# ablab/spades

Hardware: NVIDIA H100
Metric: Mk-mers/s (extract+count+index) k=55, 150 bp reads (higher is better)
Workload: dtype u64

## Files before the change

spades_b200/csrc/count.cu:

```cuda
#include <time.h>

#include <algorithm>
#include <type_traits>

#include "sgpu_internal.h"

namespace sg {

struct ReadsSrc {
    const uint64_t *words;
    const uint64_t *offs;
    const uint32_t *lens;
    int64_t n;
    uint64_t nwords;
    int K;
    int both;
    __device__ __forceinline__ uint32_t nrec(int64_t item) const {
        int L = (int)lens[item];
        uint32_t w = L >= K ? (uint32_t)(L - K + 1) : 0u;
        return both ? 2u * w : w;
    }
    template <int NW, typename Ptr>
    __device__ __forceinline__ Kmer<NW> get_at(Ptr s, uint32_t j) const {
        uint32_t pos = both ? (j >> 1) : j;
// ... 285 lines not shown
        __syncthreads();
    }
    for (uint32_t i = threadIdx.x; i < p.PA; i += blockDim.x) mybase[i] = cur_base[i] + cnt[i];
}

static const int kRollC = 24;
static_assert(kRollC <= 33 && kRollC % 8 == 0, "roll_init fetches a chunk's bases from two words; an id row is a whole number of 16-byte words");
static const int kRollThreads = 512;

static const int kRollTile = 32;
static const int kRollWarps = kRollThreads / 32;
static const int kRollStageWords = 320;
__device__ __forceinline__ void prefetch_l2(const void *p) { asm volatile("prefetch.global.L2 [%0];" ::"l"(p)); }
struct RollWarp {
    uint64_t words[kRollStageWords];
    uint32_t pref[kRollTile + 1];
    uint32_t len[kRollTile];
    uint32_t off[kRollTile];
    uint32_t pad_;
};
static_assert(sizeof(RollWarp) % 8 == 0, "per-warp slices stay 8-byte aligned");
static size_t roll_smem_bytes(uint32_t nslots) { return (((size_t)nslots * 4 + 15) & ~(size_t)15) + (size_t)kRollWarps * sizeof(RollWarp); }
__device__ __forceinline__ RollWarp *roll_warp_slice(unsigned char *raw, uint32_t nslots) {
    return reinterpret_cast<RollWarp *>(raw + (((size_t)nslots * 4 + 15) & ~(size_t)15)) + (threadIdx.x >> 5);
}

__device__ __forceinline__ uint32_t roll_warp_setup(const ReadsSrc &src, int64_t item0, int nitems, RollWarp &rw, uint32_t *uniform, bool *staged) {
    const int lane = threadIdx.x & 31;
    uint32_t c = 0, L = 0;
    uint64_t a = 0, b = 0;
    if (lane < nitems) {
        L = src.lens[item0 + lane];
        a = src.offs[item0 + lane];
        b = a + (((uint64_t)L + 31) >> 5);
        const uint32_t w = (int)L >= src.K ? (uint32_t)((int)L - src.K + 1) : 0u;
        c = (w + kRollC - 1) / kRollC;
    }
    uint32_t inc = c;
#pragma unroll
    for (int o = 1; o < 32; o <<= 1) {
        const uint32_t t = __shfl_up_sync(0xffffffffu, inc, o);
        if (lane >= o) inc += t;
    }
    rw.len[lane] = L;
    rw.pref[lane] = inc - c;
    const uint32_t total = __shfl_sync(0xffffffffu, inc, 31);
    if (lane == 31) rw.pref[kRollTile] = total;
    const uint32_t c0 = __shfl_sync(0xffffffffu, c, 0);
    const bool same = __all_sync(0xffffffffu, lane >= nitems || c == c0);
    *uniform = (same && c0) ? c0 : 0u;
    const uint64_t w0 = __shfl_sync(0xffffffffu, a, 0);
    const bool ok = lane >= nitems || (a >= w0 && b >= a && b - w0 <= (uint64_t)kRollStageWords);
    const bool st = __all_sync(0xffffffffu, ok);
    if (st) {
        rw.off[lane] = (uint32_t)(a - w0);
        uint32_t end = lane < nitems ? (uint32_t)(b - w0) : 0u;
#pragma unroll
        for (int o = 16; o; o >>= 1) end = max(end, __shfl_xor_sync(0xffffffffu, end, o));
        uint64_t tmp[kRollStageWords / 32];
#pragma unroll
        for (int j = 0; j < kRollStageWords / 32; ++j) tmp[j] = (uint32_t)(lane + 32 * j) < end ? __ldg(src.words + w0 + lane + 32 * j) : 0ull;
#pragma unroll
        for (int j = 0; j < kRollStageWords / 32; ++j) if ((uint32_t)(lane + 32 * j) < end) rw.words[lane + 32 * j] = tmp[j];
    }
    *staged = st;
    __syncwarp();
    return total;
}

__global__ void roll_tile_ids_k(ReadsSrc src, int64_t ntiles, uint32_t *__restrict__ out) {
    const int64_t t = (int64_t)blockIdx.x * (blockDim.x >> 5) + (threadIdx.x >> 5);
    if (t >= ntiles) return;
    const int lane = threadIdx.x & 31;
    const int64_t item = t * kRollTile + lane;
    uint32_t s = 0;
    if (item < src.n) {
        const int L = (int)src.lens[item];
        const uint32_t w = L >= src.K ? (uint32_t)(L - src.K + 1) : 0u;
        s = (w + kRollC - 1) / kRollC;
    }
    for (int o = 16; o; o >>= 1) s += __shfl_down_sync(0xffffffffu, s, o);
    if (lane == 0) out[t] = s * kRollC;
}

struct RollUnit { int it, j0, cnt; };
__device__ __forceinline__ RollUnit roll_unit(const RollWarp &rw, int nitems, uint32_t u, uint32_t unif, int K) {
    RollUnit q;
    q.it = find_item_u(rw.pref, nitems, u, unif);
    q.j0 = (int)(u - rw.pref[q.it]) * kRollC;
    const int nwin = (int)rw.len[q.it] - K + 1;
    q.cnt = nwin - q.j0 < kRollC ? nwin - q.j0 : kRollC;
    return q;
}

template <int NW>
__global__ void __launch_bounds__(kRollThreads, 2) levelA_count_roll_k(ReadsSrc src, LevelA p, uint32_t *__restrict__ blk_counts,
                                                                      const uint64_t *__restrict__ tile_off, uint16_t *__restrict__ ids) {
    extern __shared__ __align__(16) unsigned char sm_raw[];
    uint32_t *hist = reinterpret_cast<uint32_t *>(sm_raw);
    RollWarp &rw = *roll_warp_slice(sm_raw, p.PA);
    for (uint32_t i = threadIdx.x; i < p.PA; i += blockDim.x) hist[i] = 0;
    __syncthreads();
    const int K = p.K;
    const int lane = threadIdx.x & 31, warp = threadIdx.x >> 5;
    const int64_t ntiles = (src.n + kRollTile - 1) / kRollTile;
    const int64_t per = (ntiles + gridDim.x - 1) / gridDim.x;
    const int64_t t0 = (int64_t)blockIdx.x * per, t1 = min(ntiles, t0 + per);
    for (int64_t t = t0 + warp; t < t1; t += kRollWarps) {
        const int64_t item0 = t * kRollTile;
        const int nitems = (int)min((int64_t)kRollTile, src.n - item0);
        uint32_t unif = 0;
        bool staged = false;
        const bool has_next = t + kRollWarps < t1;
        const int64_t nx = (t + kRollWarps) * kRollTile;
        uint64_t next_w0 = 0;
        if (has_next) {
            next_w0 = src.offs[nx];
            if (lane == 0) prefetch_l2(src.lens + nx);
            else if (lane == 1 && nx + 16 < src.n) prefetch_l2(src.offs + nx + 16);
        }
        const uint32_t nunits = roll_warp_setup(src, item0, nitems, rw, &unif, &staged);
        uint64_t *row = ids ? reinterpret_cast<uint64_t *>(ids + tile_off[t]) : nullptr;
        for (uint32_t u = lane; u < nunits; u += 32) {
            const RollUnit q = roll_unit(rw, nitems, u, unif, K);
            const uint64_t *seq = staged ? static_cast<const uint64_t *>(rw.words + rw.off[q.it]) : src.words + src.offs[item0 + q.it];
            RollState<NW> st;
            roll_init<NW>(st, seq, q.j0, K, q.cnt);
#pragma unroll 1
            for (int g = 0; g < kRollC / 4; ++g) {
                uint64_t acc = 0;
#pragma unroll
                for (int e = 0; e < 4; ++e) {
                    const int s = 4 * g + e;
                    uint32_t id = 0xffffu;
                    if (s < q.cnt) {
                        if (s > 0) roll_next<NW>(st, K);
                        const Kmer<NW> k = kmer_is_minimal<NW>(st.f, st.r) ? st.f : st.r;
                        uint32_t part;
                        if (part_of<NW>(p, k, &part)) { atomicAdd(&hist[part], 1u); id = part; }
                    }
                    acc |= (uint64_t)id << (16 * e);
                }
                if (row) row[(size_t)u * (kRollC / 4) + g] = acc;
            }
        }
        if (has_next && lane < 10 && next_w0 + 16 * lane < src.nwords) prefetch_l2(src.words + next_w0 + 16 * lane);
        __syncwarp();
    }
    __syncthreads();
    uint32_t *out = blk_counts + (size_t)blockIdx.x * p.PA;
    for (uint32_t i = threadIdx.x; i < p.PA; i += blockDim.x) out[i] += hist[i];
}

template <int NW, bool HAS_IDS>
__global__ void __launch_bounds__(kRollThreads, 2) levelA_scatter_roll_k(ReadsSrc src, LevelA p, uint64_t *__restrict__ base, uint64_t *__restrict__ out,
                                                                        const uint64_t *__restrict__ tile_off, const uint16_t *__restrict__ ids,
                                                                        uint32_t id_lo, uint32_t row_stride, uint32_t q_lo, uint64_t ids_len) {
    extern __shared__ __align__(16) unsigned char sm_raw[];
    uint32_t *cur = reinterpret_cast<uint32_t *>(sm_raw);
    RollWarp &rw = *roll_warp_slice(sm_raw, p.PA);
    uint64_t *mybase = base + (size_t)blockIdx.x * row_stride + q_lo;
    const uint64_t region0 = mybase[0];
    for (uint32_t i = threadIdx.x; i < p.PA; i += blockDim.x) cur[i] = (uint32_t)(mybase[i] - region0);
    __syncthreads();
    uint64_t *const out0 = out + region0 * NW;
    const int K = p.K;
    const uint32_t PA = p.PA;
    const int lane = threadIdx.x & 31, warp = threadIdx.x >> 5;
    const int64_t ntiles = (src.n + kRollTile - 1) / kRollTile;
    const int64_t per = (ntiles + gridDim.x - 1) / gridDim.x;
    const int64_t t0 = (int64_t)blockIdx.x * per, t1 = min(ntiles, t0 + per);
    for (int64_t t = t0 + warp; t < t1; t += kRollWarps) {
        const int64_t item0 = t * kRollTile;
        const int nitems = (int)min((int64_t)kRollTile, src.n - item0);
        uint32_t unif = 0;
        bool staged = false;
        const bool has_next = t + kRollWarps < t1;
        const int64_t nx = (t + kRollWarps) * kRollTile;
        uint64_t next_w0 = 0;
        if (has_next) {
            next_w0 = src.offs[nx];
            if (lane == 0) prefetch_l2(src.lens + nx);
            else if (lane == 1 && nx + 16 < src.n) prefetch_l2(src.offs + nx + 16);
        }
        uint64_t next_row = 0;
        if (HAS_IDS && has_next) next_row = tile_off[t + kRollWarps];
        const uint32_t nunits = roll_warp_setup(src, item0, nitems, rw, &unif, &staged);
        const ulonglong2 *row = HAS_IDS ? reinterpret_cast<const ulonglong2 *>(ids + tile_off[t]) : nullptr;
        for (uint32_t u = lane; u < nunits; u += 32) {
            uint64_t idw[kRollC / 4];
            if (HAS_IDS) {
#pragma unroll
                for (int v = 0; v < kRollC / 8; ++v) {
                    const ulonglong2 x = __ldg(row + (size_t)u * (kRollC / 8) + v);
                    idw[2 * v] = x.x; idw[2 * v + 1] = x.y;
                }
            }
            const RollUnit q = roll_unit(rw, nitems, u, unif, K);
            const uint64_t *seq = staged ? static_cast<const uint64_t *>(rw.words + rw.off[q.it]) : src.words + src.offs[item0 + q.it];
            RollState<NW> st;
            roll_init<NW>(st, seq, q.j0, K, q.cnt);
#pragma unroll
            for (int s = 0; s < kRollC; ++s) {
                if (s >= q.cnt) break;
                if (s > 0) roll_next<NW>(st, K);
                uint32_t part;
                bool mine;
                if (HAS_IDS) {
                    part = (uint32_t)((idw[s >> 2] >> (16 * (s & 3))) & 0xffffu) - id_lo;
                    mine = part < PA;
                    if (mine) {
                        const uint32_t slot = atomicAdd(&cur[part], 1u);
                        const bool fwd = kmer_is_minimal<NW>(st.f, st.r);
                        Kmer<NW> k;
#pragma unroll
                        for (int j = 0; j < NW; ++j) k.w[j] = fwd ? st.f.w[j] : st.r.w[j];
                        store_rec_stream<NW>(out0 + (size_t)slot * NW, k);
                    }
                } else {
                    const Kmer<NW> k = kmer_is_minimal<NW>(st.f, st.r) ? st.f : st.r;
                    mine = part_of<NW>(p, k, &part);
                    if (mine) {
                        const uint32_t slot = atomicAdd(&cur[part], 1u);
                        store_rec_stream<NW>(out0 + (size_t)slot * NW, k);
                    }
                }
            }
        }
        if (has_next && lane < 10 && next_w0 + 16 * lane < src.nwords) prefetch_l2(src.words + next_w0 + 16 * lane);
        if (HAS_IDS && has_next) {
            if (next_row + 64 * lane < ids_len) prefetch_l2(ids + next_row + 64 * lane);
            if (lane < 16 && next_row + 64 * (32 + lane) < ids_len) prefetch_l2(ids + next_row + 64 * (32 + lane));
        }
        __syncwarp();
    }
    __syncthreads();
    for (uint32_t i = threadIdx.x; i < PA; i += blockDim.x) mybase[i] = region0 + cur[i];
}


struct Seg {
    uint64_t start;
    uint64_t len;
    uint32_t bits;
    uint32_t bb;
};

__global__ void seg_init_k(const uint64_t *__restrict__ part_start, const uint64_t *__restrict__ part_total, uint32_t PA, int rA,
                           uint32_t b_lo, Seg *__restrict__ segs) {
    uint32_t part = blockIdx.x * blockDim.x + threadIdx.x;
    if (part >= PA) return;
    Seg s;
    s.start = part_start[part]; s.len = part_total[part]; s.bits = (uint32_t)rA; s.bb = ((b_lo + (part >> rA)) << 1) | 0u;
    segs[part] = s;
}

struct Pieces {
    const uint64_t *pbase;
    const uint32_t *cnt;
    uint32_t cnt_stride, PA;
    int G;
};
static const int kMaxPieces = 1024;

__global__ void stage_rows_k(const uint32_t *__restrict__ cnt, uint32_t cnt_stride, uint32_t PA, uint64_t *__restrict__ rel, uint64_t *__restrict__ row_total) {
    __shared__ uint64_t wsum[8];
    __shared__ uint64_t carry_s;
    const uint32_t *row = cnt + (size_t)blockIdx.x * cnt_stride;
    uint64_t *out = rel + (size_t)blockIdx.x * PA;
    const int lane = threadIdx.x & 31, warp = threadIdx.x >> 5;
    if (threadIdx.x == 0) carry_s = 0;
    __syncthreads();
    for (uint32_t b = 0; b < PA; b += blockDim.x) {
        const uint32_t i = b + threadIdx.x;
        const uint64_t v = i < PA ? row[i] : 0;
        uint64_t inc = v;
#pragma unroll
        for (int o = 1; o < 32; o <<= 1) {
            uint64_t t = __shfl_up_sync(0xffffffffu, inc, o);
            if (lane >= o) inc += t;
        }
        if (lane == 31) wsum[warp] = inc;
        __syncthreads();
        uint64_t wb = 0, all = 0;
        for (int w = 0; w < 8; ++w) { if (w < warp) wb += wsum[w]; all += wsum[w]; }
        const uint64_t carry = carry_s;
        if (i < PA) out[i] = carry + wb + inc - v;
        __syncthreads();
        if (threadIdx.x == 0) carry_s = carry + all;
        __syncthreads();
    }
    if (threadIdx.x == 0) row_total[blockIdx.x] = carry_s;
}
__global__ void stage_add_k(uint64_t *__restrict__ rel, const uint64_t *__restrict__ row_start, uint32_t PA, int G) {
    const uint64_t i = (uint64_t)blockIdx.x * blockDim.x + threadIdx.x;
    if (i >= (uint64_t)G * PA) return;
    rel[i] += row_start[i / PA];
}

struct RefinePlan { uint32_t cap, target, rmax; int total_bits; };
__device__ __forceinline__ int plan_r(const RefinePlan &rp, uint64_t len, uint32_t bits) {
    if (len <= rp.cap) return 0;
    int rem = rp.total_bits - (int)bits;
    if (rem <= 0) return 0;
    uint64_t want = (len + rp.target - 1) / rp.target;
    int r = 1;
    while (r < (int)rp.rmax && (1ull << r) < want) ++r;
    return r < rem ? r : rem;
}
__global__ void refine_plan_k(const Seg *__restrict__ segs, uint64_t n, RefinePlan rp, uint32_t *__restrict__ nchild, uint32_t *__restrict__ isw, int force_all) {
    uint64_t i = (uint64_t)blockIdx.x * blockDim.x + threadIdx.x;
    if (i >= n) return;
    int r = plan_r(rp, segs[i].len, segs[i].bits);
    nchild[i] = r ? (1u << r) : 1u;
    isw[i] = (r || force_all) ? 1u : 0u;
}
__global__ void refine_copy_k(const Seg *__restrict__ segs, uint64_t n, const uint32_t *__restrict__ isw, const uint64_t *__restrict__ child_base,
                              const uint64_t *__restrict__ work_pos, Seg *__restrict__ nsegs, uint64_t *__restrict__ worklist) {
    uint64_t i = (uint64_t)blockIdx.x * blockDim.x + threadIdx.x;
    if (i >= n) return;
    if (isw[i]) worklist[work_pos[i]] = i;
    else nsegs[child_base[i]] = segs[i];
}

static const int kRThreads = 1024;
static const int kRWarps = kRThreads / 32;
static const int kRMaxBins = 2048;
template <int NW> struct RBatch {
    static const int RPT = NW == 1 ? 12 : NW == 2 ? 8 : NW == 3 ? 4 : 3;
    static const int N = RPT * kRThreads;
    static constexpr size_t smem() { return (size_t)N * (NW * sizeof(uint64_t) + sizeof(uint32_t)); }
};

template <int NW, bool PIECED>
__global__ void __launch_bounds__(kRThreads) refine_k(const Seg *__restrict__ segs, const uint64_t *__restrict__ worklist, uint64_t nwork,
                                                     const uint64_t *__restrict__ child_base, RefinePlan rp, int K,
                                                     uint64_t *__restrict__ buf0, uint64_t *__restrict__ buf1, Seg *__restrict__ nsegs,
                                                     unsigned long long *__restrict__ work_counter, Pieces pc) {
    constexpr int RPT = RBatch<NW>::RPT, N = RBatch<NW>::N;
    __shared__ uint32_t hist[kRMaxBins];
    __shared__ uint32_t run_off[kRMaxBins];
    __shared__ uint32_t run_slot[kRMaxBins];
    __shared__ uint32_t warp_tot[kRWarps];
    __shared__ unsigned long long s_w;
    __shared__ uint64_t pc_start[PIECED ? kMaxPieces : 1];
    __shared__ uint32_t pc_len[PIECED ? kMaxPieces : 1];
    extern __shared__ uint64_t sm_refine_dyn[];
    uint64_t *stage = sm_refine_dyn;
    uint32_t *stage_slot = reinterpret_cast<uint32_t *>(stage + (size_t)N * NW);
    const int lane = threadIdx.x & 31, warp = threadIdx.x >> 5;
    for (;;) {
        if (threadIdx.x == 0) s_w = atomicAdd(work_counter, 1ull);
        __syncthreads();
        const uint64_t wi = s_w;
        __syncthreads();
        if (wi >= nwork) return;
        const uint64_t si = worklist[wi];
        const Seg s = segs[si];
        const int r = plan_r(rp, s.len, s.bits);
        const uint32_t nb = 1u << r;
        const uint64_t *src = ((s.bb & 1) ? buf1 : buf0) + s.start * NW;
        uint64_t *dst = ((s.bb & 1) ? buf0 : buf1) + s.start * NW;
        if (PIECED) {
            for (int g = threadIdx.x; g < pc.G; g += blockDim.x) {
                pc_start[g] = pc.pbase[(size_t)g * pc.PA + si];
                pc_len[g] = pc.cnt[(size_t)g * pc.cnt_stride + si];
            }
        }
        for (uint32_t i = threadIdx.x; i < nb; i += blockDim.x) hist[i] = 0;
        __syncthreads();
        if (PIECED) {
            for (int g = warp; g < pc.G; g += kRWarps) {
                const uint64_t *ps = buf0 + pc_start[g] * NW;
                const uint32_t n = pc_len[g];
                uint32_t i = lane;
                for (; i + 96 < n; i += 128) {
                    const Kmer<NW> k0 = load_rec<NW>(ps + (uint64_t)i * NW), k1 = load_rec<NW>(ps + (uint64_t)(i + 32) * NW);
                    const Kmer<NW> k2 = load_rec<NW>(ps + (uint64_t)(i + 64) * NW), k3 = load_rec<NW>(ps + (uint64_t)(i + 96) * NW);
                    atomicAdd(&hist[key_bits<NW>(k0, K, (int)s.bits, r)], 1u);
                    atomicAdd(&hist[key_bits<NW>(k1, K, (int)s.bits, r)], 1u);
                    atomicAdd(&hist[key_bits<NW>(k2, K, (int)s.bits, r)], 1u);
                    atomicAdd(&hist[key_bits<NW>(k3, K, (int)s.bits, r)], 1u);
                }
                for (; i < n; i += 32) {
                    const Kmer<NW> k = load_rec<NW>(ps + (uint64_t)i * NW);
                    atomicAdd(&hist[key_bits<NW>(k, K, (int)s.bits, r)], 1u);
                }
            }
        } else {
            for (uint64_t i = threadIdx.x; i < s.len; i += blockDim.x) {
                Kmer<NW> k = load_rec<NW>(src + i * NW);
                atomicAdd(&hist[key_bits<NW>(k, K, (int)s.bits, r)], 1u);
// ... 478 lines not shown
        if (const char *e = getenv("SGPU_RMAX")) x.rmax = (uint32_t)std::min(11, std::max(1, atoi(e)));
        if (const char *e = getenv("SGPU_A_SUB")) x.a_sub = std::min(64, std::max(0, atoi(e)));
        x.trace = getenv("SGPU_TRACE") != nullptr;
        return x;
    }();
    return t;
}

struct Trace {
    bool on; cudaStream_t st; double t0;
    static double now() { struct timespec ts; clock_gettime(CLOCK_MONOTONIC, &ts); return ts.tv_sec * 1e3 + ts.tv_nsec * 1e-6; }
    Trace(cudaStream_t s) : on(tuning().trace), st(s), t0(now()) {}
    void mark(const char *what) {
        if (!on) return;
        cudaStreamSynchronize(st);
        double t = now();
        fprintf(stderr, "[sgpu-trace] %-28s %9.3f ms\n", what, t - t0);
        t0 = t;
    }
};

static int ilog2_floor(uint64_t v) { int r = 0; while (v >>= 1) ++r; return r; }

static const int kLevelAMaxParts = 8192;

template <int NW> static uint32_t sort_target() { return (uint32_t)SortCfg<NW>::CAP * 6 / 8; }

template <int NW>
static void sort_pass(Ctx *ctx, int K, DArr<uint64_t> &X, DArr<uint64_t> &Y, const uint64_t *part_start_p, const uint64_t *part_total_p, uint32_t PA,
                      int rA_, uint32_t b_lo, int b_hi, int64_t first, bool want_counts, bool double_selfrc, unsigned long long *d_bsz_p, Chunk &ch_out,
                      Timer &tm, Trace &tr, const Pieces *pieces = nullptr) {
    constexpr int CAP = SortCfg<NW>::CAP;
    const int total_bits = 2 * K;
    cudaStream_t st = ctx->stream;
    uint64_t nsegs = PA;
    DArr<Seg> segs(ctx, nsegs);
    seg_init_k<<<div_up(PA, 256), 256, 0, st>>>(part_start_p, part_total_p, PA, rA_, b_lo, segs.p);
    ctx->launches++;
    RefinePlan rp; rp.cap = CAP; rp.target = sort_target<NW>(); rp.total_bits = total_bits;
    rp.rmax = tuning().rmax;
    DArr<unsigned long long> wcounter(ctx, 4);
    tm.start();
    uint64_t rounds = 0;
    for (int round = 0; round < 300; ++round) {
        DArr<uint32_t> nchild(ctx, nsegs + 1), isw(ctx, nsegs + 1);
        DArr<uint64_t> cbase(ctx, nsegs + 1), wpos(ctx, nsegs + 1);
        SG_CUDA(cudaMemsetAsync(nchild.p + nsegs, 0, 4, st));
        SG_CUDA(cudaMemsetAsync(isw.p + nsegs, 0, 4, st));
        const bool pieced = pieces && round == 0;
        refine_plan_k<<<div_up(nsegs, 256), 256, 0, st>>>(segs.p, nsegs, rp, nchild.p, isw.p, pieced ? 1 : 0);
        ctx->launches++;
        exclusive_scan_u32_to_u64(ctx, nchild.p, cbase.p, nsegs + 1);
        exclusive_scan_u32_to_u64(ctx, isw.p, wpos.p, nsegs + 1);
        uint64_t tot[2];
        SG_CUDA(cudaMemcpyAsync(&tot[0], cbase.p + nsegs, 8, cudaMemcpyDeviceToHost, st));
        SG_CUDA(cudaMemcpyAsync(&tot[1], wpos.p + nsegs, 8, cudaMemcpyDeviceToHost, st));
        SG_CUDA(cudaStreamSynchronize(st));
        if (tot[1] == 0) break;
        DArr<Seg> nsegs_arr(ctx, tot[0]);
        DArr<uint64_t> worklist(ctx, tot[1]);
        refine_copy_k<<<div_up(nsegs, 256), 256, 0, st>>>(segs.p, nsegs, isw.p, cbase.p, wpos.p, nsegs_arr.p, worklist.p);
        ctx->launches++;
        SG_CUDA(cudaMemsetAsync(wcounter.p, 0, 8, st));
        const int grid = (int)std::min<uint64_t>(tot[1], (uint64_t)ctx->num_sms);
        const size_t sm = RBatch<NW>::smem();
        if (pieced) {
            SG_CUDA(cudaFuncSetAttribute(refine_k<NW, true>, cudaFuncAttributeMaxDynamicSharedMemorySize, (int)sm));
            refine_k<NW, true><<<grid, kRThreads, sm, st>>>(segs.p, worklist.p, tot[1], cbase.p, rp, K, X.p, Y.p, nsegs_arr.p, wcounter.p, *pieces);
        } else {
            SG_CUDA(cudaFuncSetAttribute(refine_k<NW, false>, cudaFuncAttributeMaxDynamicSharedMemorySize, (int)sm));
            refine_k<NW, false><<<grid, kRThreads, sm, st>>>(segs.p, worklist.p, tot[1], cbase.p, rp, K, X.p, Y.p, nsegs_arr.p, wcounter.p, Pieces());
        }
        ctx->launches++;
        SG_CUDA(cudaGetLastError());
        tr.mark("refine round");
        (round == 0 ? ctx->times.refine_splits_round0 : ctx->times.refine_splits_later) += tot[0] - nsegs;
        ++rounds;
        segs = std::move(nsegs_arr);
        nsegs = tot[0];
    }
    ctx->times.refine_rounds_max = std::max(ctx->times.refine_rounds_max, rounds);
    ctx->times.refine += tm.stop();
    DArr<uint32_t> ndist(ctx, nsegs + 1);
    DArr<unsigned long long> stats(ctx, 4);
    SG_CUDA(cudaMemsetAsync(ndist.p, 0, ndist.bytes(), st));
    SG_CUDA(cudaMemsetAsync(stats.p, 0, 32, st));
    SG_CUDA(cudaMemsetAsync(wcounter.p, 0, 8, st));
    tm.start();
    {
        auto launch = [&](auto kernel, size_t smem) {
            SG_CUDA(cudaFuncSetAttribute(kernel, cudaFuncAttributeMaxDynamicSharedMemorySize, (int)smem));
            int occ = 1;
            SG_CUDA(cudaOccupancyMaxActiveBlocksPerMultiprocessor(&occ, kernel, kSThreads, smem));
            if (occ < 1) occ = 1;
            int grid = (int)std::min<uint64_t>(nsegs, (uint64_t)ctx->num_sms * occ);
            if (grid < 1) grid = 1;
            kernel<<<grid, kSThreads, smem, st>>>(segs.p, nsegs, K, X.p, Y.p, ndist.p, wcounter.p, stats.p);
        };
        constexpr int bins = 1 << kSortBinBits;
        launch(local_sort3_k<NW, kSortBinBits, CAP>, (size_t)(CAP + kResCap) * NW * sizeof(uint64_t) + (size_t)3 * bins * sizeof(uint32_t) +
                                                         ((size_t)2 * bins + 2 + kResCap) * sizeof(uint16_t) + 16);
        ctx->launches++;
        SG_CUDA(cudaGetLastError());
    }
    DArr<uint64_t> dbase(ctx, nsegs + 1);
    exclusive_scan_u32_to_u64(ctx, ndist.p, dbase.p, nsegs + 1);
    uint64_t D = 0;
    unsigned long long h_stats[4];
    SG_CUDA(cudaMemcpyAsync(&D, dbase.p + nsegs, 8, cudaMemcpyDeviceToHost, st));
    SG_CUDA(cudaMemcpyAsync(h_stats, stats.p, 32, cudaMemcpyDeviceToHost, st));
    SG_CUDA(cudaStreamSynchronize(st));
    ctx->times.local_sort += tm.stop();
    tr.mark("local sort");
    SG_CHECK(h_stats[0] == 0, 6, "internal: oversize segment with unfixed key bits reached the local sort");
    ctx->times.sort_lsd_fallbacks += h_stats[1];
    ctx->times.sort_oversize_equal += h_stats[2];
    Chunk ch;
    ch.n = (int64_t)D; ch.b_lo = (int)b_lo; ch.b_hi = b_hi; ch.first = first;
    ch.keys.alloc(ctx, (size_t)D * NW + 2, true);
    if (want_counts) ch.counts.alloc(ctx, (size_t)D + 1, true);
    tm.start();
    if (nsegs) {
        compact_k<NW><<<div_up((int64_t)nsegs * 32, 256), 256, 0, st>>>(segs.p, nsegs, ndist.p, dbase.p, X.p, Y.p, K, want_counts ? 1 : 0,
                                                                     double_selfrc ? 1 : 0, ch.keys.p, ch.counts.p, d_bsz_p);
        ctx->launches++;
        SG_CUDA(cudaGetLastError());
    }
    ctx->times.compact += tm.stop();
    tr.mark("compact");
    ch_out = std::move(ch);
}

template <int NW, class Src>
struct LevelAJob {
    Ctx *ctx = nullptr;
    std::vector<Src> srcs;
    int K = 0, B = 0, rA = 0, G = 0;
    int s_lo = 0, s_hi = 0;
    uint32_t PA_all = 0;
    bool roll = false, use_ids = false;
    DArr<uint32_t> blk_counts;
    DArr<uint64_t> part_total_all;
    std::vector<DArr<uint64_t>> tile_off;
    std::vector<DArr<uint16_t>> ids;
    std::vector<uint64_t> h_part;
    uint64_t bucket_records(int b) const {
        uint64_t s = 0;
        for (uint32_t q = 0; q < (1u << rA); ++q) s += h_part[((size_t)(b - s_lo) << rA) + q];
        return s;
    }
};

static int levelA_ctas_per_sm() { return 2; }
static int levelA_key_bits(uint64_t est_records, int B, int total_bits, uint32_t target, uint32_t pa_max) {
    const int want = ilog2_floor(est_records / target + 1) + 1;
    const int bbits = ilog2_floor((uint64_t)B) + (((1u << ilog2_floor((uint64_t)B)) < (uint32_t)B) ? 1 : 0);
    int rA = want - bbits;
    if (rA < 0) rA = 0;
    while (rA > 0 && ((uint64_t)B << rA) > pa_max) --rA;
    if (rA > total_bits) rA = total_bits;
    if (rA > 13) rA = 13;
    return rA;
}

template <int NW, class Src>
static void levelA_count(LevelAJob<NW, Src> &job, uint64_t est_records, Timer &tm, Trace &tr) {
    Ctx *ctx = job.ctx;
    cudaStream_t st = ctx->stream;
    const uint32_t PA_all = job.PA_all;
    const int G = job.G;
    SG_CHECK(PA_all >= 1 && PA_all <= (uint32_t)kLevelAMaxParts, 6, "internal: level-A partition table too large");
    LevelA pa_all;
    pa_all.K = job.K; pa_all.B = (uint32_t)job.B; pa_all.b_lo = (uint32_t)job.s_lo; pa_all.b_hi = (uint32_t)job.s_hi; pa_all.rA = job.rA; pa_all.PA = PA_all;
    job.blk_counts.alloc(ctx, (size_t)G * PA_all);
    job.part_total_all.alloc(ctx, (size_t)PA_all + 1);
    job.h_part.assign(PA_all, 0);
    SG_CUDA(cudaMemsetAsync(job.blk_counts.p, 0, job.blk_counts.bytes(), st));
    job.tile_off.clear(); job.ids.clear();
    job.tile_off.resize(job.srcs.size()); job.ids.resize(job.srcs.size());
    job.use_ids = PA_all < 0xffffu && (double)est_records * 2.0 < (double)ctx->free_bytes() * 0.20;
    if (job.use_ids) {
        for (size_t si = 0; si < job.srcs.size(); ++si) {
            const Src &src = job.srcs[si];
            if (src.n == 0) continue;
            const int64_t ntiles = (src.n + (job.roll ? kRollTile : kATile) - 1) / (job.roll ? kRollTile : kATile);
            DArr<uint32_t> ttot(ctx, (size_t)ntiles + 1);
            job.tile_off[si].alloc(ctx, (size_t)ntiles + 1);
            SG_CUDA(cudaMemsetAsync(ttot.p + ntiles, 0, 4, st));
            if (job.roll) {
                if constexpr (std::is_same<Src, ReadsSrc>::value) roll_tile_ids_k<<<div_up(ntiles, 8), 256, 0, st>>>(src, ntiles, ttot.p);
            } else {
                tile_totals_k<Src><<<div_up(ntiles, 8), 256, 0, st>>>(src, ntiles, ttot.p, 8u);
            }
            ctx->launches++;
            exclusive_scan_u32_to_u64(ctx, ttot.p, job.tile_off[si].p, (size_t)ntiles + 1);
            uint64_t nrec_src = 0;
            SG_CUDA(cudaMemcpyAsync(&nrec_src, job.tile_off[si].p + ntiles, 8, cudaMemcpyDeviceToHost, st));
            SG_CUDA(cudaStreamSynchronize(st));
            job.ids[si].alloc(ctx, (size_t)nrec_src + 8);
        }
    }
    tm.start();
    for (size_t si = 0; si < job.srcs.size(); ++si) {
        const Src &src = job.srcs[si];
        if (src.n == 0) continue;
        if (job.roll) {
            if constexpr (std::is_same<Src, ReadsSrc>::value) {
                SG_CUDA(cudaFuncSetAttribute(levelA_count_roll_k<NW>, cudaFuncAttributeMaxDynamicSharedMemorySize, (int)roll_smem_bytes(PA_all)));
                levelA_count_roll_k<NW><<<G, kRollThreads, roll_smem_bytes(PA_all), st>>>(src, pa_all, job.blk_counts.p, job.tile_off[si].p, job.ids[si].p);
            }
        } else {
            SG_CUDA(cudaFuncSetAttribute(levelA_count_k<NW, Src>, cudaFuncAttributeMaxDynamicSharedMemorySize, (int)(PA_all * sizeof(uint32_t))));
            levelA_count_k<NW, Src><<<G, kAThreads, PA_all * sizeof(uint32_t), st>>>(src, pa_all, job.blk_counts.p, job.tile_off[si].p, job.ids[si].p);
        }
        ctx->launches++;
    }
    SG_CUDA(cudaGetLastError());
    levelA_totals_k<<<div_up(PA_all, 256), 256, 0, st>>>(job.blk_counts.p, PA_all, G, job.part_total_all.p);
    ctx->launches++;
    SG_CUDA(cudaMemcpyAsync(job.h_part.data(), job.part_total_all.p, (size_t)PA_all * 8, cudaMemcpyDeviceToHost, st));
    SG_CUDA(cudaStreamSynchronize(st));
    ctx->times.extract_count += tm.stop();
    tr.mark("A1 count+totals");
}

template <int NW, class Src>
static void levelA_scatter(LevelAJob<NW, Src> &job, int b_lo, int b_hi, uint64_t I_pass, uint64_t total_records, uint64_t *X, uint64_t *pbase_buf,
                           Pieces &pcs, Timer &tm, Trace &tr) {
    Ctx *ctx = job.ctx;
    cudaStream_t st = ctx->stream;
    const int G = job.G;
    const uint32_t PA_all = job.PA_all;
    const uint32_t p_lo = (uint32_t)(b_lo - job.s_lo) << job.rA;
    LevelA pa;
    pa.K = job.K; pa.B = (uint32_t)job.B; pa.b_lo = (uint32_t)b_lo; pa.b_hi = (uint32_t)b_hi; pa.rA = job.rA; pa.PA = (uint32_t)(b_hi - b_lo) << job.rA;
    const uint32_t PA = pa.PA;
    SG_CHECK(PA >= 1 && PA <= (uint32_t)kLevelAMaxParts && G <= kMaxPieces, 6, "internal: level-A pass geometry");
    DArr<uint64_t> base(ctx, (size_t)G * PA);
    {
        DArr<uint64_t> row_total(ctx, (size_t)G + 1), row_start(ctx, (size_t)G + 1);
        SG_CUDA(cudaMemsetAsync(row_total.p + G, 0, 8, st));
        stage_rows_k<<<G, 256, 0, st>>>(job.blk_counts.p + p_lo, PA_all, PA, base.p, row_total.p);
        exclusive_scan_u64(ctx, row_total.p, row_start.p, (size_t)G + 1);
        stage_add_k<<<div_up((int64_t)G * PA, 256), 256, 0, st>>>(base.p, row_start.p, PA, G);
        ctx->launches += 2;
        SG_CUDA(cudaMemcpyAsync(pbase_buf, base.p, (size_t)G * PA * 8, cudaMemcpyDeviceToDevice, st));
    }
    pcs.pbase = pbase_buf; pcs.cnt = job.blk_counts.p + p_lo; pcs.cnt_stride = PA_all; pcs.PA = PA; pcs.G = G;
    tm.start();
    if (job.roll) {
        if constexpr (std::is_same<Src, ReadsSrc>::value) {
            const size_t smem = roll_smem_bytes(PA);
            SG_CUDA(cudaFuncSetAttribute(levelA_scatter_roll_k<NW, true>, cudaFuncAttributeMaxDynamicSharedMemorySize, (int)smem));
            SG_CUDA(cudaFuncSetAttribute(levelA_scatter_roll_k<NW, false>, cudaFuncAttributeMaxDynamicSharedMemorySize, (int)smem));
            {
            int nsub_auto = (int)(4.0 * (double)I_pass / (double)std::max<uint64_t>(1, total_records) + 0.5);
            nsub_auto = std::min(4, std::max(1, nsub_auto));
            uint32_t nsub = job.use_ids ? (uint32_t)(tuning().a_sub ? tuning().a_sub : nsub_auto) : 1u;
            if (nsub > PA) nsub = PA;
            for (uint32_t sb = 0; sb < nsub; ++sb) {
                const uint32_t q_lo = (uint32_t)((uint64_t)PA * sb / nsub), q_hi = (uint32_t)((uint64_t)PA * (sb + 1) / nsub);
                if (q_hi == q_lo) continue;
                LevelA pa_sub = pa;
                pa_sub.PA = q_hi - q_lo;
                const size_t smem_sub = roll_smem_bytes(pa_sub.PA);
                for (size_t si = 0; si < job.srcs.size(); ++si) {
                    const Src &src = job.srcs[si];
                    if (src.n == 0) continue;
                    if (job.use_ids)
                        levelA_scatter_roll_k<NW, true><<<G, kRollThreads, smem_sub, st>>>(src, pa_sub, base.p, X, job.tile_off[si].p, job.ids[si].p, p_lo + q_lo, PA, q_lo, (uint64_t)job.ids[si].n);
                    else
                        levelA_scatter_roll_k<NW, false><<<G, kRollThreads, smem, st>>>(src, pa, base.p, X, nullptr, nullptr, 0u, PA, 0u, 0ull);
                    ctx->launches++; ctx->times.level_a_scatters++;
                }
            }
            }
        }
    } else {
        const size_t smem = (size_t)PA * (sizeof(uint64_t) + sizeof(uint32_t));
        SG_CUDA(cudaFuncSetAttribute(levelA_scatter_k<NW, Src>, cudaFuncAttributeMaxDynamicSharedMemorySize, (int)smem));
        for (size_t si = 0; si < job.srcs.size(); ++si) {
            const Src &src = job.srcs[si];
            if (src.n == 0) continue;
            levelA_scatter_k<NW, Src><<<G, kAThreads, smem, st>>>(src, pa, base.p, X, job.use_ids ? job.tile_off[si].p : nullptr,
                                                                 job.use_ids ? job.ids[si].p : nullptr, p_lo);
            ctx->launches++; ctx->times.level_a_scatters++;
        }
    }
    SG_CUDA(cudaGetLastError());
    ctx->times.extract_scatter += tm.stop();
    tr.mark("A2 scatter");
}

static double pass_bytes_needed(uint64_t recs, size_t W) { return (double)recs * W * 2.0 + (double)recs * (W + 4) * 0.6 + (64 << 20); }

template <int NW, class Src>
static void run_count(Ctx *ctx, const std::vector<Src> &srcs, int K, int B, bool want_counts, bool double_selfrc, uint64_t est_records, KSet *out) {
    const int total_bits = 2 * K;
    const size_t W = 8 * NW;
    cudaStream_t st = ctx->stream;
    Timer tm(st);
    Trace tr(st);
    constexpr bool kIsReads = std::is_same<Src, ReadsSrc>::value;

    out->bsz.assign(B, 0);
    DArr<unsigned long long> d_bsz(ctx, B);
    SG_CUDA(cudaMemsetAsync(d_bsz.p, 0, B * sizeof(unsigned long long), st));

    const int rA = levelA_key_bits(est_records, B, total_bits, sort_target<NW>(), tuning().pa_max);
    ctx->times.level_a_key_bits = (uint64_t)rA;
    const int SR = std::max(1, kLevelAMaxParts >> rA);
    const int n_ranges = (B + SR - 1) / SR;
    int64_t first = 0;
    for (int s_lo = 0; s_lo < B; s_lo += SR) {
        const int share = (kMaxChunks - (int)out->chunks.size()) / (n_ranges - s_lo / SR);
        LevelAJob<NW, Src> job;
        job.ctx = ctx; job.srcs = srcs; job.K = K; job.B = B; job.rA = rA; job.G = ctx->num_sms * levelA_ctas_per_sm();
        job.s_lo = s_lo; job.s_hi = std::min(B, s_lo + SR);
        job.PA_all = (uint32_t)(job.s_hi - job.s_lo) << rA;
        if constexpr (kIsReads) job.roll = !srcs.empty() && !srcs[0].both;
        levelA_count(job, est_records, tm, tr);
        auto current_limit = [&]() {
            return ctx->hbm_budget ? (ctx->hbm_budget > ctx->allocated ? ctx->hbm_budget - ctx->allocated : 0) : (size_t)(ctx->free_bytes() * 0.90);
        };
        uint64_t total_records = 0;
        for (int b = job.s_lo; b < job.s_hi; ++b) total_records += job.bucket_records(b);
        uint64_t pass_target = total_records;
        bool capped = false;
        {
            double lim_sim = (double)current_limit();
            int npass_sim = 0, b = job.s_lo;
            while (b < job.s_hi) {
                uint64_t I = 0; const int b0 = b;
                while (b < job.s_hi) {
                    const uint64_t ib = job.bucket_records(b);
                    if (b > b0 && pass_bytes_needed(I + ib, W) > lim_sim) break;
                    I += ib; ++b;
                }
                lim_sim -= (double)I * (W + 4) * 0.5;
                ++npass_sim;
            }
            capped = npass_sim > share;
            pass_target = total_records / (uint64_t)std::min(npass_sim, share) + total_records / 64 + 1;
        }
        int b_lo = job.s_lo, npass = 0;
        while (b_lo < job.s_hi) {
            const int left = share - npass;
            const int min_b = (capped || left == 1) ? div_up(job.s_hi - b_lo, left) : 1;
            const size_t lim = current_limit();
            int b_hi = b_lo;
            uint64_t I = 0;
            while (b_hi < job.s_hi) {
                const uint64_t ib = job.bucket_records(b_hi);
                if (b_hi - b_lo >= min_b && (pass_bytes_needed(I + ib, W) > (double)lim || I + ib > pass_target)) break;
                I += ib; ++b_hi;
            }
            ++npass;
            const uint32_t p_lo = (uint32_t)(b_lo - job.s_lo) << rA;
            const uint32_t PA = (uint32_t)(b_hi - b_lo) << rA;
            DArr<uint64_t> part_total(ctx, PA + 1), part_start(ctx, PA + 1);
            SG_CUDA(cudaMemcpyAsync(part_total.p, job.part_total_all.p + p_lo, (size_t)PA * 8, cudaMemcpyDeviceToDevice, st));
            SG_CUDA(cudaMemsetAsync(part_total.p + PA, 0, 8, st));
            exclusive_scan_u64(ctx, part_total.p, part_start.p, PA + 1);
            ctx->times.passes++;
            ctx->times.instances += I;
            DArr<uint64_t> X(ctx, (size_t)I * NW + 2), Y(ctx, (size_t)I * NW + 2);
            DArr<uint64_t> pbase(ctx, (size_t)job.G * PA);
            Pieces pcs;
            levelA_scatter(job, b_lo, b_hi, I, total_records, X.p, pbase.p, pcs, tm, tr);
            Chunk ch;
            sort_pass<NW>(ctx, K, X, Y, part_start.p, part_total.p, PA, rA, (uint32_t)b_lo, b_hi, first, want_counts, double_selfrc, d_bsz.p, ch, tm, tr, &pcs);
            first += ch.n;
            out->chunks.push_back(std::move(ch));
            b_lo = b_hi;
        }
    }
    std::vector<unsigned long long> hb(B);
    SG_CUDA(cudaMemcpyAsync(hb.data(), d_bsz.p, B * sizeof(unsigned long long), cudaMemcpyDeviceToHost, st));
    SG_CUDA(cudaStreamSynchronize(st));
    out->bstart.assign(B + 1, 0);
    for (int b = 0; b < B; ++b) { out->bsz[b] = (int64_t)hb[b]; out->bstart[b + 1] = out->bstart[b] + out->bsz[b]; }
    out->n = first;
    SG_CHECK(out->bstart[B] == out->n, 6, "internal: bucket sizes do not add up");
}

__global__ void count_windows_k(const uint32_t *__restrict__ lens, int64_t n, int K, unsigned long long *__restrict__ out) {
    unsigned long long s = 0;
    for (int64_t i = (int64_t)blockIdx.x * blockDim.x + threadIdx.x; i < n; i += (int64_t)gridDim.x * blockDim.x) {
        int L = (int)lens[i];
        if (L >= K) s += (unsigned long long)(L - K + 1);
    }
    for (int o = 16; o; o >>= 1) s += __shfl_down_sync(0xffffffffu, s, o);
    if ((threadIdx.x & 31) == 0 && s) atomicAdd(out, s);
}

static uint64_t count_windows(Ctx *ctx, int K) {
    DArr<unsigned long long> d_w(ctx, 1);
    SG_CUDA(cudaMemsetAsync(d_w.p, 0, 8, ctx->stream));
    if (ctx->n_reads) {
        count_windows_k<<<ctx->num_sms * 4, 256, 0, ctx->stream>>>(ctx->d_lens, ctx->n_reads, K, d_w.p);
        ctx->launches++;
    }
    unsigned long long wn = 0;
    SG_CUDA(cudaMemcpyAsync(&wn, d_w.p, 8, cudaMemcpyDeviceToHost, ctx->stream));
    SG_CUDA(cudaStreamSynchronize(ctx->stream));
    return (uint64_t)wn;
}

static ReadsSrc reads_source(Ctx *ctx, int K, bool both) {
    ReadsSrc src;
    src.words = ctx->d_words; src.offs = ctx->d_offs; src.lens = ctx->d_lens; src.n = ctx->n_reads; src.nwords = ctx->n_words; src.K = K; src.both = both;
    return src;
}

template <int NW>
static KSet *count_reads_nw(Ctx *ctx, int K, int B, int mode) {
    ensure_reads_on_device(ctx);
    KSet *ks = new KSet();
    ks->ctx = ctx; ks->K = K; ks->nw = NW; ks->B = B; ks->has_counts = (mode == kCanonical);
    try {
        const bool both = (mode == kAllWindows);
        const uint64_t wn = count_windows(ctx, K);
        std::vector<ReadsSrc> srcs{reads_source(ctx, K, both)};
        run_count<NW, ReadsSrc>(ctx, srcs, K, B, mode == kCanonical, mode == kCanonical && (K % 2 == 0), wn * (both ? 2 : 1), ks);
    } catch (...) { delete ks; throw; }
// ... 501 lines not shown
```

Baseline: 7142.

## Stage level-A scatter records in shared memory and flush sorted by partition

The rolling level-A scatter kernel no longer writes each k-mer straight to its partition slot in global memory. Records are now collected in a shared-memory batch with warp-aggregated fill counters. When the batch fills, the block runs a prefix scan over per-partition counts, sorts the staged records by partition, and writes them out so consecutive threads target contiguous slots. The aim is coalesced global stores in place of scattered ones, at the cost of a restructured warp state machine, extra block-wide syncs, and much larger shared-memory use that could lower occupancy.

```diff
diff --git a/spades_b200/csrc/count.cu b/spades_b200/csrc/count.cu
--- a/spades_b200/csrc/count.cu
+++ b/spades_b200/csrc/count.cu
@@ -461,92 +461,186 @@
     for (uint32_t i = threadIdx.x; i < p.PA; i += blockDim.x) out[i] += hist[i];
 }
 
+static const uint32_t kABatchNoTag = 0xffffffffu;
+static const int kABatchPartBits = 13;
+static const uint32_t kABatchMin = 1024;
+template <int NW> struct ABatch {
+    static constexpr size_t rec_bytes() { return NW * sizeof(uint64_t) + sizeof(uint32_t) + sizeof(uint16_t); }
+};
+__host__ __device__ __forceinline__ size_t abatch_offset(uint32_t PA) {
+    return ((((size_t)2 * PA * 4 + 15) & ~(size_t)15) + (size_t)kRollWarps * sizeof(RollWarp) + 15) & ~(size_t)15;
+}
+
 template <int NW, bool HAS_IDS>
 __global__ void __launch_bounds__(kRollThreads, 2) levelA_scatter_roll_k(ReadsSrc src, LevelA p, uint64_t *__restrict__ base, uint64_t *__restrict__ out,
                                                                         const uint64_t *__restrict__ tile_off, const uint16_t *__restrict__ ids,
-                                                                        uint32_t id_lo, uint32_t row_stride, uint32_t q_lo, uint64_t ids_len) {
+                                                                        uint32_t id_lo, uint32_t row_stride, uint32_t q_lo, uint64_t ids_len, uint32_t cap) {
     extern __shared__ __align__(16) unsigned char sm_raw[];
+    __shared__ uint32_t s_fill;
+    __shared__ uint32_t warp_tot[kRollWarps];
+    const uint32_t PA = p.PA;
     uint32_t *cur = reinterpret_cast<uint32_t *>(sm_raw);
-    RollWarp &rw = *roll_warp_slice(sm_raw, p.PA);
+    uint32_t *cnt = cur + PA;
+    RollWarp &rw = *roll_warp_slice(sm_raw, 2 * PA);
+    uint64_t *stage = reinterpret_cast<uint64_t *>(sm_raw + abatch_offset(PA));
+    uint32_t *tags = reinterpret_cast<uint32_t *>(stage + (size_t)cap * NW);
+    uint16_t *idx = reinterpret_cast<uint16_t *>(tags + cap);
     uint64_t *mybase = base + (size_t)blockIdx.x * row_stride + q_lo;
     const uint64_t region0 = mybase[0];
-    for (uint32_t i = threadIdx.x; i < p.PA; i += blockDim.x) cur[i] = (uint32_t)(mybase[i] - region0);
+    for (uint32_t i = threadIdx.x; i < PA; i += blockDim.x) { cur[i] = (uint32_t)(mybase[i] - region0); cnt[i] = 0; }
+    if (threadIdx.x == 0) s_fill = 0;
     __syncthreads();
     uint64_t *const out0 = out + region0 * NW;
     const int K = p.K;
-    const uint32_t PA = p.PA;
     const int lane = threadIdx.x & 31, warp = threadIdx.x >> 5;
+    const uint32_t lt_mask = (1u << lane) - 1u;
     const int64_t ntiles = (src.n + kRollTile - 1) / kRollTile;
     const int64_t per = (ntiles + gridDim.x - 1) / gridDim.x;
     const int64_t t0 = (int64_t)blockIdx.x * per, t1 = min(ntiles, t0 + per);
-    for (int64_t t = t0 + warp; t < t1; t += kRollWarps) {
-        const int64_t item0 = t * kRollTile;
-        const int nitems = (int)min((int64_t)kRollTile, src.n - item0);
-        uint32_t unif = 0;
-        bool staged = false;
-        const bool has_next = t + kRollWarps < t1;
-        const int64_t nx = (t + kRollWarps) * kRollTile;
-        uint64_t next_w0 = 0;
-        if (has_next) {
-            next_w0 = src.offs[nx];
-            if (lane == 0) prefetch_l2(src.lens + nx);
-            else if (lane == 1 && nx + 16 < src.n) prefetch_l2(src.offs + nx + 16);
-        }
-        uint64_t next_row = 0;
-        if (HAS_IDS && has_next) next_row = tile_off[t + kRollWarps];
-        const uint32_t nunits = roll_warp_setup(src, item0, nitems, rw, &unif, &staged);
-        const ulonglong2 *row = HAS_IDS ? reinterpret_cast<const ulonglong2 *>(ids + tile_off[t]) : nullptr;
-        for (uint32_t u = lane; u < nunits; u += 32) {
-            uint64_t idw[kRollC / 4];
-            if (HAS_IDS) {
-#pragma unroll
-                for (int v = 0; v < kRollC / 8; ++v) {
-                    const ulonglong2 x = __ldg(row + (size_t)u * (kRollC / 8) + v);
-                    idw[2 * v] = x.x; idw[2 * v + 1] = x.y;
-                }
-            }
-            const RollUnit q = roll_unit(rw, nitems, u, unif, K);
-            const uint64_t *seq = staged ? static_cast<const uint64_t *>(rw.words + rw.off[q.it]) : src.words + src.offs[item0 + q.it];
-            RollState<NW> st;
-            roll_init<NW>(st, seq, q.j0, K, q.cnt);
-#pragma unroll
-            for (int s = 0; s < kRollC; ++s) {
-                if (s >= q.cnt) break;
-                if (s > 0) roll_next<NW>(st, K);
-                uint32_t part;
-                bool mine;
+
+    int64_t t = t0 + warp;
+    bool need_setup = true;
+    int nitems = 0;
+    uint32_t nunits = 0, unif = 0;
+    bool staged = false;
+    uint64_t next_w0 = 0, next_row = 0;
+    const ulonglong2 *row = nullptr;
+    int u = 0, s = 0, cnt_w = 0;
+    RollState<NW> st;
+    uint64_t idq[kRollC / 4];
+    for (;;) {
+        while (t < t1) {
+            if (need_setup) {
+                const int64_t item0 = t * kRollTile;
+                nitems = (int)min((int64_t)kRollTile, src.n - item0);
+                const int64_t nx = (t + kRollWarps) * kRollTile;
+                if (t + kRollWarps < t1) {
+                    next_w0 = src.offs[nx];
+                    if (lane == 0) prefetch_l2(src.lens + nx);
+                    else if (lane == 1 && nx + 16 < src.n) prefetch_l2(src.offs + nx + 16);
+                    if (HAS_IDS) next_row = tile_off[t + kRollWarps];
+                }
+                nunits = roll_warp_setup(src, item0, nitems, rw, &unif, &staged);
+                if (HAS_IDS) row = reinterpret_cast<const ulonglong2 *>(ids + tile_off[t]);
+                u = lane - 32; s = cnt_w = 0;
+                need_setup = false;
+            }
+            if (s >= cnt_w && u < (int)nunits) {
+                u += 32;
+                if (u < (int)nunits) {
+                    if (HAS_IDS) {
+#pragma unroll
+                        for (int v = 0; v < kRollC / 8; ++v) {
+                            const ulonglong2 x = __ldg(row + (size_t)u * (kRollC / 8) + v);
+                            idq[2 * v] = x.x; idq[2 * v + 1] = x.y;
+                        }
+                    }
+                    const RollUnit q = roll_unit(rw, nitems, (uint32_t)u, unif, K);
+                    const uint64_t *seq = staged ? static_cast<const uint64_t *>(rw.words + rw.off[q.it]) : src.words + src.offs[t * kRollTile + q.it];
+                    roll_init<NW>(st, seq, q.j0, K, q.cnt);
+                    s = 0; cnt_w = q.cnt;
+                }
+            }
+            const bool act = s < cnt_w;
+            if (!__any_sync(0xffffffffu, act)) {
+                if (t + kRollWarps < t1) {
+                    if (lane < 10 && next_w0 + 16 * lane < src.nwords) prefetch_l2(src.words + next_w0 + 16 * lane);
+                    if (HAS_IDS) {
+                        if (next_row + 64 * lane < ids_len) prefetch_l2(ids + next_row + 64 * lane);
+                        if (lane < 16 && next_row + 64 * (32 + lane) < ids_len) prefetch_l2(ids + next_row + 64 * (32 + lane));
+                    }
+                }
+                __syncwarp();
+                t += kRollWarps;
+                need_setup = true;
+                continue;
+            }
+            uint32_t part = 0;
+            bool mine = false;
+            Kmer<NW> k;
+            if (act) {
                 if (HAS_IDS) {
-                    part = (uint32_t)((idw[s >> 2] >> (16 * (s & 3))) & 0xffffu) - id_lo;
+                    part = (uint32_t)(idq[0] & 0xffffu) - id_lo;
                     mine = part < PA;
-                    if (mine) {
-                        const uint32_t slot = atomicAdd(&cur[part], 1u);
-                        const bool fwd = kmer_is_minimal<NW>(st.f, st.r);
-                        Kmer<NW> k;
-#pragma unroll
-                        for (int j = 0; j < NW; ++j) k.w[j] = fwd ? st.f.w[j] : st.r.w[j];
-                        store_rec_stream<NW>(out0 + (size_t)slot * NW, k);
+                }
+                if (!HAS_IDS || mine) {
+                    const bool fwd = kmer_is_minimal<NW>(st.f, st.r);
+#pragma unroll
+                    for (int j = 0; j < NW; ++j) k.w[j] = fwd ? st.f.w[j] : st.r.w[j];
+                }
+                if (!HAS_IDS) mine = part_of<NW>(p, k, &part);
+            }
+            const uint32_t bal = __ballot_sync(0xffffffffu, mine);
+            if (bal) {
+                const uint32_t n = __popc(bal);
+                uint32_t b0 = 0;
+                if (lane == 0) b0 = atomicAdd(&s_fill, n);
+                b0 = __shfl_sync(0xffffffffu, b0, 0);
+                if (b0 + n > cap) {
+                    if (b0 < cap && (uint32_t)lane < cap - b0) tags[b0 + lane] = kABatchNoTag;
+                    break;
+                }
+                if (mine) {
+                    const uint32_t i = b0 + __popc(bal & lt_mask);
+                    const uint32_t rank = atomicAdd(&cnt[part], 1u) & 0xffffu;
+                    store_rec<NW>(stage + (size_t)i * NW, k);
+                    tags[i] = (rank << kABatchPartBits) | part;
+                }
+            }
+            if (act && ++s < cnt_w) {
+                roll_next<NW>(st, K);
+                if (HAS_IDS) {
+                    if ((s & 3) == 0) {
+#pragma unroll
+                        for (int v = 0; v + 1 < kRollC / 4; ++v) idq[v] = idq[v + 1];
+                    } else {
+                        idq[0] >>= 16;
                     }
-                } else {
-                    const Kmer<NW> k = kmer_is_minimal<NW>(st.f, st.r) ? st.f : st.r;
-                    mine = part_of<NW>(p, k, &part);
-                    if (mine) {
-                        const uint32_t slot = atomicAdd(&cur[part], 1u);
-                        store_rec_stream<NW>(out0 + (size_t)slot * NW, k);
-                    }
-                }
-            }
-        }
-        if (has_next && lane < 10 && next_w0 + 16 * lane < src.nwords) prefetch_l2(src.words + next_w0 + 16 * lane);
-        if (HAS_IDS && has_next) {
-            if (next_row + 64 * lane < ids_len) prefetch_l2(ids + next_row + 64 * lane);
-            if (lane < 16 && next_row + 64 * (32 + lane) < ids_len) prefetch_l2(ids + next_row + 64 * (32 + lane));
-        }
-        __syncwarp();
-    }
-    __syncthreads();
+                }
+            }
+        }
+        const bool more = __syncthreads_or(t < t1);
+        const uint32_t nslots = min(s_fill, cap);
+        const uint32_t own = (PA + kRollThreads - 1) / kRollThreads;
+        const uint32_t j0 = min(PA, threadIdx.x * own), j1 = min(PA, j0 + own);
+        uint32_t sum = 0;
+        for (uint32_t j = j0; j < j1; ++j) sum += cnt[j] & 0xffffu;
+        uint32_t inc = sum;
+#pragma unroll
+        for (int o = 1; o < 32; o <<= 1) {
+            const uint32_t v = __shfl_up_sync(0xffffffffu, inc, o);
+            if (lane >= o) inc += v;
+        }
+        if (lane == 31) warp_tot[warp] = inc;
+        __syncthreads();
+        uint32_t wb = 0, total = 0;
+#pragma unroll
+        for (int w = 0; w < kRollWarps; ++w) { const uint32_t v = warp_tot[w]; if (w < warp) wb += v; total += v; }
+        uint32_t o = wb + inc - sum;
+        for (uint32_t j = j0; j < j1; ++j) {
+            const uint32_t c = cnt[j] & 0xffffu;
+            o += c;
+            cnt[j] = o << 16;
+            cur[j] += c;
+        }
+        if (threadIdx.x == 0) s_fill = 0;
+        __syncthreads();
+        for (uint32_t i = threadIdx.x; i < nslots; i += kRollThreads) {
+            const uint32_t tg = tags[i];
+            if (tg == kABatchNoTag) continue;
+            idx[(cnt[tg & ((1u << kABatchPartBits) - 1)] >> 16) - 1 - (tg >> kABatchPartBits)] = (uint16_t)i;
+        }
+        __syncthreads();
+        for (uint32_t q = threadIdx.x; q < total; q += kRollThreads) {
+            const uint32_t i = idx[q], tg = tags[i];
+            const uint32_t slot = cur[tg & ((1u << kABatchPartBits) - 1)] - 1 - (tg >> kABatchPartBits);
+            store_rec_stream<NW>(out0 + (size_t)slot * NW, load_rec<NW>(stage + (size_t)i * NW));
+        }
+        __syncthreads();
+        if (!more) break;
+    }
     for (uint32_t i = threadIdx.x; i < PA; i += blockDim.x) mybase[i] = region0 + cur[i];
 }
-
 
 struct Seg {
     uint64_t start;
@@ -1331,6 +1425,21 @@
 };
 
 static int levelA_ctas_per_sm() { return 2; }
+template <int NW>
+static size_t levelA_batch_smem(uint32_t PA, uint32_t *cap) {
+    static_assert(kLevelAMaxParts <= (1 << kABatchPartBits), "a batch tag holds the partition");
+    int dev = 0, per_sm = 0, per_cta = 0, reserved = 0;
+    SG_CUDA(cudaGetDevice(&dev));
+    SG_CUDA(cudaDeviceGetAttribute(&per_sm, cudaDevAttrMaxSharedMemoryPerMultiprocessor, dev));
+    SG_CUDA(cudaDeviceGetAttribute(&per_cta, cudaDevAttrMaxSharedMemoryPerBlockOptin, dev));
+    SG_CUDA(cudaDeviceGetAttribute(&reserved, cudaDevAttrReservedSharedMemoryPerBlock, dev));
+    const size_t rec = ABatch<NW>::rec_bytes(), fixed = abatch_offset(PA), kStatic = 128;
+    size_t room = (size_t)per_sm / levelA_ctas_per_sm() - (size_t)reserved - kStatic;
+    if (room < fixed + kABatchMin * rec) room = (size_t)per_cta - kStatic;
+    SG_CHECK(room >= fixed + kABatchMin * rec, 6, "internal: level-A batch does not fit shared memory");
+    *cap = (uint32_t)std::min<size_t>((room - fixed) / rec, 32768) & ~31u;
+    return fixed + (size_t)*cap * rec;
+}
 static int levelA_key_bits(uint64_t est_records, int B, int total_bits, uint32_t target, uint32_t pa_max) {
     const int want = ilog2_floor(est_records / target + 1) + 1;
     const int bbits = ilog2_floor((uint64_t)B) + (((1u << ilog2_floor((uint64_t)B)) < (uint32_t)B) ? 1 : 0);
@@ -1429,9 +1538,6 @@
     tm.start();
     if (job.roll) {
         if constexpr (std::is_same<Src, ReadsSrc>::value) {
-            const size_t smem = roll_smem_bytes(PA);
-            SG_CUDA(cudaFuncSetAttribute(levelA_scatter_roll_k<NW, true>, cudaFuncAttributeMaxDynamicSharedMemorySize, (int)smem));
-            SG_CUDA(cudaFuncSetAttribute(levelA_scatter_roll_k<NW, false>, cudaFuncAttributeMaxDynamicSharedMemorySize, (int)smem));
             {
             int nsub_auto = (int)(4.0 * (double)I_pass / (double)std::max<uint64_t>(1, total_records) + 0.5);
             nsub_auto = std::min(4, std::max(1, nsub_auto));
@@ -1442,14 +1548,17 @@
                 if (q_hi == q_lo) continue;
                 LevelA pa_sub = pa;
                 pa_sub.PA = q_hi - q_lo;
-                const size_t smem_sub = roll_smem_bytes(pa_sub.PA);
+                uint32_t cap = 0;
+                const size_t smem = levelA_batch_smem<NW>(pa_sub.PA, &cap);
+                if (job.use_ids) SG_CUDA(cudaFuncSetAttribute(levelA_scatter_roll_k<NW, true>, cudaFuncAttributeMaxDynamicSharedMemorySize, (int)smem));
+                else SG_CUDA(cudaFuncSetAttribute(levelA_scatter_roll_k<NW, false>, cudaFuncAttributeMaxDynamicSharedMemorySize, (int)smem));
                 for (size_t si = 0; si < job.srcs.size(); ++si) {
                     const Src &src = job.srcs[si];
                     if (src.n == 0) continue;
                     if (job.use_ids)
-                        levelA_scatter_roll_k<NW, true><<<G, kRollThreads, smem_sub, st>>>(src, pa_sub, base.p, X, job.tile_off[si].p, job.ids[si].p, p_lo + q_lo, PA, q_lo, (uint64_t)job.ids[si].n);
+                        levelA_scatter_roll_k<NW, true><<<G, kRollThreads, smem, st>>>(src, pa_sub, base.p, X, job.tile_off[si].p, job.ids[si].p, p_lo + q_lo, PA, q_lo, (uint64_t)job.ids[si].n, cap);
                     else
-                        levelA_scatter_roll_k<NW, false><<<G, kRollThreads, smem, st>>>(src, pa, base.p, X, nullptr, nullptr, 0u, PA, 0u, 0ull);
+                        levelA_scatter_roll_k<NW, false><<<G, kRollThreads, smem, st>>>(src, pa, base.p, X, nullptr, nullptr, 0u, PA, 0u, 0ull, cap);
                     ctx->launches++; ctx->times.level_a_scatters++;
                 }
             }
```

Result: faster. 8059 (median of 6 runs) (+12.8%).
